# CC834/Heterogeneous-OpenCL-Image-Processing-Engine

Measured on AMD Instinct MI355X. Metric: images_per_sec, higher is better.
Workload: dtype u8

## Files before the change

heterogeneous-opencl-image-processing-engine_amd/__init__.py:

```python
from __future__ import annotations

import ctypes as C
import os
import re
import subprocess

PKG_DIR = os.path.dirname(os.path.abspath(__file__))
ROOT = os.path.dirname(PKG_DIR)
CSRC = os.path.join(PKG_DIR, "csrc")
APPS = os.path.join(PKG_DIR, "apps")
LIB_PATH = os.path.join(PKG_DIR, "libmi_blur.so")
HEADER = os.path.join(ROOT, "include", "mi_blur.h")
HIPCC = os.environ.get("HIPCC", "/opt/rocm/bin/hipcc")
os.environ.setdefault("HIP_FORCE_DEV_KERNARG", "0")
ARCH = "gfx950"

DEVICE_CPU = -1
VARIANT_AUTO, VARIANT_GENERIC, VARIANT_TILED, VARIANT_STREAM, VARIANT_DIRECT = 0, 1, 2, 3, 4
OK, ERR_INVALID, ERR_NO_DEVICE, ERR_NOMEM, ERR_STATE, ERR_UNSUPPORTED = 0, -1, -2, -3, -4, -5
UNIQUE_ID_BYTES = 128
SEP_MAX_RADIUS = 16
MEDIAN_MAX_RADIUS = 7
MORPH_MAX_RADIUS = 16
MORPH_ERODE, MORPH_DILATE, MORPH_GRADIENT = 0, 1, 2
# ... 319 lines not shown
        "mi_blur_warp_perspective_quad": (i, [C.POINTER(C.c_double), C.POINTER(C.c_double), C.POINTER(C.c_double)]),
        "mi_blur_warp_perspective_set_matrix": (i, [C.POINTER(WarpPerspective), C.POINTER(C.c_double), i]),
        "mi_blur_enqueue_warp_perspective": (i, [u8p, u8p, i, i, i, i, C.POINTER(WarpPerspective), vp]),
        "mi_blur_cpu_run_warp_perspective": (i, [u8p, u8p, i, i, i, i, C.POINTER(WarpPerspective), i]),
        "mi_blur_ctx_set_warp_perspective": (i, [vp, C.POINTER(WarpPerspective)]),
        "mi_blur_conv_preset": (i, [i, C.POINTER(Conv)]),
        "mi_blur_enqueue_conv": (i, [u8p, u8p, i, i, i, i, C.POINTER(Conv), vp]),
        "mi_blur_enqueue_conv_band": (i, [u8p, u8p, i, i, i, i, i, C.POINTER(Conv), vp]),
        "mi_blur_cpu_run_conv": (i, [u8p, u8p, i, i, i, i, C.POINTER(Conv), i]),
        "mi_blur_ctx_set_conv": (i, [vp, C.POINTER(Conv)]),
        "mi_blur_fill_synthetic": (None, [u8p, i, i, i, i, i, i]),
        "mi_blur_fnv1a64": (C.c_uint64, [u8p, C.c_size_t]),
        "mi_blur_debug_zc_trace": (i, [vp, C.POINTER(C.c_uint64), i, C.POINTER(i), C.POINTER(C.c_uint)]),
        "mi_blur_debug_xcd_times": (i, [C.POINTER(C.c_uint64), C.POINTER(C.c_uint64), i]),
        "mi_blur_debug_xcd_raw": (i, [C.POINTER(C.c_uint64), C.c_size_t, C.c_size_t]),
        "mi_blur_a1_partition": (None, [i, i, C.c_float, C.POINTER(i), C.POINTER(i)]),
        "mi_blur_shard_range": (None, [C.c_longlong, i, i, C.POINTER(C.c_longlong), C.POINTER(C.c_longlong)]),
        "mi_blur_a2_split": (None, [i, C.c_float, i, C.POINTER(A2Geometry)]),
        "mi_blur_band_of": (None, [i, i, i, i, C.POINTER(Band)]),
        "mi_blur_comm_unique_id": (i, [vp]),
        "mi_blur_comm_init_rank": (i, [C.POINTER(vp), i, i, vp]),
        "mi_blur_comm_init_all": (i, [C.POINTER(vp), i, C.POINTER(i)]),
        "mi_blur_comm_init_p2p": (i, [C.POINTER(vp), i, C.POINTER(i)]),
        "mi_blur_comm_init_pull": (i, [C.POINTER(vp), i, C.POINTER(i)]),
        "mi_blur_comm_destroy": (None, [vp]),
        "mi_blur_comm_info": (i, [vp, C.POINTER(i), C.POINTER(i), C.POINTER(i)]),
        "mi_blur_halo_exchange": (i, [vp, u8p, i, i, i, i, vp]),
        "mi_blur_peer_export": (i, [vp, vp, C.POINTER(C.c_uint64)]),
        "mi_blur_peer_open": (i, [vp, C.c_uint64, C.POINTER(vp)]),
        "mi_blur_peer_close": (i, [vp, C.c_uint64]),
# ... 471 lines not shown
```

heterogeneous-opencl-image-processing-engine_amd/csrc/blur_kernels.hip:

```cpp
#include "kernel_common.h"

#include <math.h>
#include <stdlib.h>
#include <string.h>
#include <mutex>
#include <algorithm>

namespace mi_blur {

__device__ __forceinline__ u16x2 as_pk(uint32_t x) { return __builtin_bit_cast(u16x2, x); }
__device__ __forceinline__ uint32_t as_u32(u16x2 x) { return __builtin_bit_cast(uint32_t, x); }

constexpr uint32_t EVEN_MASK = 0x00ff00ffu;
__device__ __forceinline__ uint32_t even_of(uint32_t x) { return x & EVEN_MASK; }
__device__ __forceinline__ uint32_t odd_of(uint32_t x) { return __builtin_amdgcn_perm(0u, x, 0x0c030c01u); }
__device__ __forceinline__ uint32_t mad6(uint32_t c, uint32_t t) { return as_u32(as_pk(c) * (unsigned short)6 + as_pk(t)); }

constexpr uint32_t sel_left(int C, int q)
{
    uint32_t s = 0;
    for (int j = 0; j < 4; j++) {
        int p = -4 * q + j;
        int idx = ((p % C) + C) % C;
        s |= (uint32_t)idx << (8 * j);
// ... 118 lines not shown
        h[0] = hsum_raw<C, R, 0, 0>(w); h[1] = hsum_raw<C, R, 0, 1>(w);
        h[2] = hsum_raw<C, R, 0, 2>(w); h[3] = hsum_raw<C, R, 0, 3>(w);
        h[4] = hsum_raw<C, R, 1, 0>(w); h[5] = hsum_raw<C, R, 1, 1>(w);
        h[6] = hsum_raw<C, R, 1, 2>(w); h[7] = hsum_raw<C, R, 1, 3>(w);
        return;
    }
    uint32_t Ew[8], Ow[8];
#pragma unroll
    for (int j = 0; j < 8; j++) { Ew[j] = even_of(w[j]); Ow[j] = odd_of(w[j]); }
    h[0] = hsum<C, R, 0, 0>(Ew, Ow); h[1] = hsum<C, R, 0, 1>(Ew, Ow);
    h[2] = hsum<C, R, 0, 2>(Ew, Ow); h[3] = hsum<C, R, 0, 3>(Ew, Ow);
    h[4] = hsum<C, R, 1, 0>(Ew, Ow); h[5] = hsum<C, R, 1, 1>(Ew, Ow);
    h[6] = hsum<C, R, 1, 2>(Ew, Ow); h[7] = hsum<C, R, 1, 3>(Ew, Ow);
}

struct TiledParams {
    const uint8_t *in;
    uint8_t *out;
    long long in_stride, out_stride;
    int pitch, cpr;
    int H, y0, y1;
    int ncols, nstrips;
    int TH, ntiles_y, ngroups;
    unsigned nblocks;
    int xcd;
    int debug_copy;
    unsigned long long *xcd_times;
    int tail;
};

struct __attribute__((packed, aligned(1))) Unaligned16 { u32x4 v; };
struct __attribute__((packed, aligned(1))) Unaligned8 { u32x2 v; };
struct __attribute__((packed, aligned(1))) Unaligned4 { uint32_t v; };
struct __attribute__((packed, aligned(1))) Unaligned2 { uint16_t v; };

__device__ __forceinline__ void store16_write_through(uint8_t *q, u32x4 v);
__device__ __forceinline__ void store_chunk_ragged_wt(uint8_t *q, u32x4 v, int n);
template <bool WT = false>
__device__ __forceinline__ void store_chunk_ragged(uint8_t *q, u32x4 v, int n)
{
    if constexpr (WT) { store_chunk_ragged_wt(q, v, n); return; }
    if (n >= 16) { reinterpret_cast<Unaligned16 *>(q)->v = v; return; }
    if (n & 8) { u32x2 t; t.x = v.x; t.y = v.y; reinterpret_cast<Unaligned8 *>(q)->v = t; q += 8; v.x = v.z; v.y = v.w; }
    if (n & 4) { reinterpret_cast<Unaligned4 *>(q)->v = v.x; q += 4; v.x = v.y; }
// ... 151 lines not shown
constexpr unsigned XCD_DEBUG_SLOTS = 1u << 20;
__device__ __forceinline__ void xcd_time_mark(unsigned long long *t, unsigned long long t0)
{
    if (threadIdx.x == 0 && blockIdx.x < XCD_DEBUG_SLOTS) {
        unsigned id;
        asm volatile("s_getreg_b32 %0, hwreg(HW_REG_XCC_ID)" : "=s"(id));
        t[2u * blockIdx.x] = ((unsigned long long)__builtin_amdgcn_s_memrealtime() << 4) | (id & 7u);
        t[2u * blockIdx.x + 1] = t0;
    }
}

template <int C, int R, int RPG, bool DMA, bool SHFL = false, bool RAG = false>
__global__ __launch_bounds__(256) void blur_tiled_kernel(const TiledParams p)
{
    const unsigned long long t0 = p.xcd_times ? __builtin_amdgcn_s_memrealtime() : 0ull;
    tiled_tile<C, R, RPG, DMA, SHFL, RAG>(p, xcd_map(blockIdx.x, p.nblocks, p.xcd));
    if (p.xcd_times) xcd_time_mark(p.xcd_times, t0);
}

template <int C, int R, int RPG>
__global__ __launch_bounds__(256) void blur_tiled_loop_kernel(const TiledParams p)
{
    for (unsigned L = blockIdx.x; L < p.nblocks; L += gridDim.x) {
        tiled_tile<C, R, RPG, true, false, false>(p, L);
        __syncthreads();
    }
}

template <int C, int R, int RPG, int X>
__global__ __launch_bounds__(256) void blur_tiled_x_kernel(const TiledParams p)
{
    tiled_tile<C, R, RPG, true, false, false, false, X>(p, xcd_map(blockIdx.x, p.nblocks, p.xcd));
}

struct FusedParams {
    unsigned *count;
    unsigned kcount;
    unsigned tiles_per_batch;
    int release;
    unsigned window;
    unsigned *tail_ctr;
    unsigned nstatic, ntail, nextra;
    unsigned *gate;
    unsigned gate_block, gate_seq;
};

template <int C, int R, int RPG>
__global__ __launch_bounds__(256) void blur_fused_kernel(const TiledParams p, const FusedParams f)
{
    const unsigned tpw = f.tiles_per_batch * f.window;
    const unsigned wnd = blockIdx.x / tpw, base = wnd * tpw;
    const unsigned nw = min(tpw, p.nblocks - base);
    const unsigned w = blockIdx.x - base;
    const unsigned tile = base + (nw >= 16 ? xcd_map(w, nw, p.xcd) : w);
    const unsigned b = tile / f.tiles_per_batch;
    tiled_tile<C, R, RPG, true, false, false, true>(p, tile);
    asm volatile("s_waitcnt vmcnt(0)" ::: "memory");
    __syncthreads();
    if (threadIdx.x == 0) {
        if (f.release) __hip_atomic_fetch_add(&f.count[b * f.kcount + ((w ^ (w >> 3)) & (f.kcount - 1u))], 1u, __ATOMIC_RELEASE, __HIP_MEMORY_SCOPE_AGENT);
        else __hip_atomic_fetch_add(&f.count[b * f.kcount + ((w ^ (w >> 3)) & (f.kcount - 1u))], 1u, __ATOMIC_RELAXED, __HIP_MEMORY_SCOPE_AGENT);
    }
}

template <int C, int R, int RPG, bool RAG = false>
__global__ __launch_bounds__(256) void blur_fused_tail_kernel(const TiledParams p, const FusedParams f)
{
    const unsigned long long t0 = p.xcd_times ? __builtin_amdgcn_s_memrealtime() : 0ull;
    if (f.gate && blockIdx.x == f.gate_block && threadIdx.x == 0) __hip_atomic_store(f.gate, f.gate_seq, __ATOMIC_RELAXED, __HIP_MEMORY_SCOPE_AGENT);
    unsigned tile, w;
    if (blockIdx.x >= f.nstatic) {
        __shared__ unsigned s_ticket;
        if (threadIdx.x == 0) {
            const unsigned t = __hip_atomic_fetch_add(f.tail_ctr, 1u, __ATOMIC_RELAXED, __HIP_MEMORY_SCOPE_AGENT);
            if (t == f.nextra - 1u) __hip_atomic_store(f.tail_ctr, 0u, __ATOMIC_RELAXED, __HIP_MEMORY_SCOPE_AGENT);
            s_ticket = t;
        }
        __syncthreads();
        const unsigned t = __builtin_amdgcn_readfirstlane(s_ticket);
        if (t >= f.ntail) return;
        tile = f.nstatic + t;
        w = t;
    } else {
        const unsigned tpw = f.tiles_per_batch * f.window;
// ... 380 lines not shown
    }
    wait_vmcnt<0>();
}

struct DirectParams {
    const uint8_t *in;
    uint8_t *out;
    long long in_stride, out_stride;
    long long total;
    int pitch, cpr;
    int H, y0, y1;
    int nbands;
    unsigned nblocks;
    int xcd;
    const uint8_t *top, *bottom;
};

template <int C, int R, int BH, bool PEER = false>
__global__ __launch_bounds__(256) void blur_direct_kernel(const DirectParams p)
{
    constexpr int WIN = 2 * R + 1, NR = BH + 2 * R;
    const int lane = threadIdx.x & 63, wave = threadIdx.x >> 6;
    const unsigned B = xcd_map(blockIdx.x, p.nblocks, p.xcd);
    const long long fl = (long long)(B * 4u + (unsigned)wave) * 62 - 1 + lane;
    const bool inrange = fl >= 0 && fl < p.total;
    const unsigned f = (unsigned)(fl < 0 ? 0 : (fl >= p.total ? p.total - 1 : fl));
    const unsigned col = f % (unsigned)p.cpr, t2 = f / (unsigned)p.cpr;
    const unsigned band = t2 % (unsigned)p.nbands;
    const long long img = (long long)(t2 / (unsigned)p.nbands);
    const bool compute = inrange && lane >= 1 && lane <= 62;
// ... 9 lines not shown
    if constexpr (PEER) outside = __builtin_amdgcn_ballot_w64(row0 - R < p.y0 || row0 + BH + R > p.y1) != 0ull;
    if (outside) {
#pragma unroll
        for (int j = 0; j < NR; j++) {
            const int sr = min(max(row0 - R + j, 0), p.H - 1);
            const uint8_t *rp = src + (size_t)sr * (size_t)p.pitch;
            if (sr < p.y0 && p.top) rp = p.top + (size_t)col * 16u + (size_t)sr * (size_t)p.pitch;
            if (sr >= p.y1 && p.bottom) rp = p.bottom + (size_t)col * 16u + (size_t)(sr - p.y1) * (size_t)p.pitch;
            rows[j] = *reinterpret_cast<const uint4 *>(rp);
        }
    } else {
#pragma unroll
        for (int j = 0; j < NR; j++)
            rows[j] = *reinterpret_cast<const uint4 *>(src + (size_t)min(max(row0 - R + j, 0), p.H - 1) * (size_t)p.pitch);
    }

    uint32_t hw[WIN][8];
#pragma unroll
    for (int j = 0; j < NR; j++) {
        uint32_t w[8];
        const uint4 c = rows[j];
        w[2] = c.x; w[3] = c.y; w[4] = c.z; w[5] = c.w;
        w[0] = __builtin_amdgcn_update_dpp(0u, c.z, 0x138, 0xf, 0xf, false);
        w[1] = __builtin_amdgcn_update_dpp(0u, c.w, 0x138, 0xf, 0xf, false);
        w[6] = __builtin_amdgcn_update_dpp(0u, c.x, 0x130, 0xf, 0xf, false);
        w[7] = __builtin_amdgcn_update_dpp(0u, c.y, 0x130, 0xf, 0xf, false);
        hrow_window<C, R, rowpass_default<R>>(w, any_edge, at_start, at_end, hw[j % WIN]);
        if (j >= 2 * R) {
            const int i = j - 2 * R;
            uint32_t o[4];
// ... 3 lines not shown
                    const uint32_t se = (((hw[(j + 2) % WIN][q] << 1) + hw[(j + 1) % WIN][q]) + hw[j % WIN][q]) << 4;
                    const uint32_t so = (((hw[(j + 2) % WIN][4 + q] << 1) + hw[(j + 1) % WIN][4 + q]) + hw[j % WIN][4 + q]) << 4;
                    o[q] = __builtin_amdgcn_perm(so, se, 0x07030501u);
                } else {
                    const uint32_t se = mad6(hw[(j + 3) % WIN][q], ((hw[(j + 2) % WIN][q] + hw[(j + 4) % WIN][q]) << 2) + (hw[(j + 1) % WIN][q] + hw[j % WIN][q]));
                    const uint32_t so = mad6(hw[(j + 3) % WIN][4 + q], ((hw[(j + 2) % WIN][4 + q] + hw[(j + 4) % WIN][4 + q]) << 2) + (hw[(j + 1) % WIN][4 + q] + hw[j % WIN][4 + q]));
                    o[q] = __builtin_amdgcn_perm(so, se, 0x07030501u);
                }
            }
            if (i < rows_out) {
                u32x4 v; v.x = o[0]; v.y = o[1]; v.z = o[2]; v.w = o[3];
                *reinterpret_cast<u32x4 *>(dst + (size_t)i * (size_t)p.pitch) = v;
            }
        }
    }
}

struct GenericParams {
    const uint8_t *in;
    uint8_t *out;
    long long in_stride, out_stride, total;
    int width, channels, pitch;
    int H, y0;
};

template <int R>
__global__ __launch_bounds__(256) void blur_generic_kernel(const GenericParams p)
{
    constexpr int T1[3] = {1, 2, 1};
    constexpr int T2[5] = {1, 4, 6, 4, 1};
// ... 167 lines not shown
    const long long nblocks = (long long)d.n_images * p.ntiles_y * p.nstrips;
    if (nblocks > 0x7fffffffLL) return MI_BLUR_ERR_INVALID;
    p.nblocks = (unsigned)nblocks;
    int xmap = 0;
    if (tun.xcd_remap && nblocks >= 16) {
        xmap = tun.xcd_run >= 2 ? tun.xcd_run : 1;
        if (xmap >= 2 && (long long)xmap * 8 > nblocks) xmap = 1;
    }
    p.xcd = xmap;
    p.debug_copy = tun.debug_copy;
    p.xcd_times = tun.debug_xcd_times ? debug_xcd_buffer() : nullptr;
    p.tail = pitch % 16 ? pitch % 16 : 16;
    *block_threads = (unsigned)((p.ncols * p.ngroups + 63) / 64 * 64);
    *lds_bytes = (size_t)(p.TH + 2 * R) * (p.ncols + 2) * 16;
    return rpg;
}

static int launch_tiled(const LaunchDesc &d, const Tunables &tun, bool ragged = false, const FusedDesc *fused = nullptr)
{
    if (!(fused && fused->geometry_only))
        g_last_kernel = fused ? "blur_fused_kernel" : (d.max_blocks > 0 && !ragged && d.channels <= 4 ? "blur_tiled_loop_kernel" : "blur_tiled_kernel");
    const int R = d.filter->radius;
    TiledParams p{};
    unsigned threads = 0;
    size_t lds = 0;
    const int rpg = tiled_geometry(d, tun, ragged, fused != nullptr, (fused && ragged) ? 8 : 0, p, &threads, &lds);
    if (rpg < 0) return rpg;
    const long long nblocks = p.nblocks;
    const dim3 grid((unsigned)nblocks), block(threads);
    if (fused) {
// ... 12 lines not shown
        if (fused->counters_per_batch) *fused->counters_per_batch = k;
        if (fused->tiles_per_batch) *fused->tiles_per_batch = (unsigned)tpb;
        if (fused->waves_per_block) *fused->waves_per_block = 1;
        if (fused->total_blocks) *fused->total_blocks = (unsigned)nblocks;
        const unsigned ntail = tun.fused_tail > 0 && fused->tail_ctr && nblocks >= 8192 ? (unsigned)(nblocks * tun.fused_tail / 1000) : 0u;
        if (fused->tail_tiles) *fused->tail_tiles = ntail >= 8 ? ntail : 0u;
        if (fused->geometry_only) return MI_BLUR_OK;
        p.debug_copy = 0;
        if (ntail >= 8) {
            f.tail_ctr = fused->tail_ctr; f.ntail = ntail; f.nstatic = (unsigned)nblocks - ntail;
            f.nextra = ntail + (unsigned)((long long)ntail * std::max(10, tun.fused_tail_blocks) / 100);
            g_last_kernel = "blur_fused_tail_kernel";
            const dim3 tgrid(f.nstatic + f.nextra);
            if (fused->gate && tun.fused_overlap > 0 && !ragged) {
                const long long ahead = nblocks * tun.fused_overlap / 1000;
                f.gate = fused->gate; f.gate_seq = fused->seq;
                f.gate_block = (unsigned)std::min<long long>(std::max<long long>(nblocks - ahead, 0), (long long)tgrid.x - 1);
            }
            if (p.xcd_times && tgrid.x <= 65536u) p.xcd_times += 2ull * 65536ull * (fused->seq & 15u);
            return dispatch<1, 2>(R, [&](auto Rc) { return launch_fused_r<Rc>(d, p, f, tgrid, block, lds, rpg, ragged); });
        }
        if (ragged) {
            if (!fused->tail_ctr) return MI_BLUR_ERR_UNSUPPORTED;
            f.tail_ctr = fused->tail_ctr; f.ntail = 0; f.nstatic = (unsigned)nblocks; f.nextra = 0;
            g_last_kernel = "blur_fused_tail_kernel";
        }
        return dispatch<1, 2>(R, [&](auto Rc) { return launch_fused_r<Rc>(d, p, f, grid, block, lds, rpg, ragged); });
    }
    return dispatch<1, 2>(R, [&](auto Rc) {
        return launch_tiled_r<Rc>(d, p, grid, block, lds, rpg, tun.stage_dma != 0, ragged, tun.row_shuffle != 0, tun.experiment);
    });
}

int zc_fill_batch(const LaunchDesc &d, ZcGeometry *geo, ZcBatch *b, unsigned *n_tiles)
{
    if (!geo || !b || !d.in || !d.out || d.n_images <= 0) return MI_BLUR_ERR_INVALID;
    Tunables tun = tunables();
    const bool aligned = tiled_eligible(d.in, d.out, d.width, d.channels) && !(d.in_stride % 16) && !(d.out_stride % 16);
    const long long pitch_b = (long long)d.width * d.channels;
    const bool dense = (!d.in_stride || d.in_stride == pitch_b * d.band_rows) && (!d.out_stride || d.out_stride == pitch_b * (d.y1 - d.y0));
    const bool ragged = !aligned && tun.ragged && ragged_eligible(d.width, d.channels) && dense;
    if (!aligned && !ragged) return MI_BLUR_ERR_UNSUPPORTED;
// ... 92 lines not shown
        return dispatch<1, 2>(d.filter->radius, [&](auto R) { return do_launch(blur_stream_kernel<C, R>, grid, block, lds, d, p); });
    });
}

template <int BH>
static int launch_direct_bh(const LaunchDesc &d, const Tunables &tun)
{
    g_last_kernel = "blur_direct_kernel";
    DirectParams p{};
    fill_band(p, d);
    p.cpr = p.pitch / 16; p.y1 = d.y1;
    const dim3 grid = direct_grid(p, d, BH), block(256);
    if (p.total >= 0x7fffffffLL) return MI_BLUR_ERR_INVALID;
    p.xcd = (tun.xcd_remap && p.nblocks >= 16) ? 1 : 0;
    const bool peer = d.halo_top || d.halo_bottom;
    if constexpr (BH != 8) {
        if (peer) return MI_BLUR_ERR_INVALID;
        return dispatch<1, 2>(d.filter->radius, [&](auto R) { return do_launch(blur_direct_kernel<3, R, BH>, grid, block, 0, d, p); });
    } else {
        if (peer) {
            p.top = d.halo_top; p.bottom = d.halo_bottom;
            g_last_kernel = "blur_direct_kernel (peer halo rows)";
            return dispatch<1, 2, 3, 4>(d.channels, [&](auto C) {
                return dispatch<1, 2>(d.filter->radius, [&](auto R) { return do_launch(blur_direct_kernel<C, R, 8, true>, grid, block, 0, d, p); });
            });
        }
        return dispatch<1, 2, 3, 4>(d.channels, [&](auto C) {
            return dispatch<1, 2>(d.filter->radius, [&](auto R) { return do_launch(blur_direct_kernel<C, R, 8>, grid, block, 0, d, p); });
        });
    }
// ... 80 lines not shown
```

heterogeneous-opencl-image-processing-engine_amd/csrc/blur_launch.h:

```cpp
#pragma once
#include <hip/hip_runtime.h>
#include <stdint.h>

#include "filter.h"

namespace mi_blur {

struct LaunchDesc {
    const Filter *filter;
    const uint8_t *in;
    uint8_t *out;
    int width, band_rows, channels;
    int n_images;
    int y0, y1;
    long long in_stride, out_stride;
    int concurrent;
    int max_blocks;
    int variant;
    const uint8_t *halo_top, *halo_bottom;
    hipStream_t stream;
    hipEvent_t start, stop;
};

int launch(const LaunchDesc &d);
int launch_sep(const LaunchDesc &d);
int launch_median(const LaunchDesc &d);
int launch_morph(const LaunchDesc &d);
int launch_bilateral(const LaunchDesc &d);
int launch_conv(const LaunchDesc &d);
int launch_sep_down(const LaunchDesc &d);
int launch_resize(const LaunchDesc &d);
int launch_warp(const LaunchDesc &d);
int launch_warp_persp(const LaunchDesc &d);
void set_last_kernel(const char *name);

struct Tunables;
// ... 60 lines not shown
    int stage_dma; int rpg; int xcd_remap; int debug_copy; int row_shuffle; int prefer_stream; int stream_bh; int zero_copy; int ragged;
    int fused_release;
    int experiment;
    int xcd_run;
    int zero_copy_streams;
    int zero_copy_blocks;
    int stream_updown;
    int prefer_direct;
    int direct_bh;
    int debug_xcd_times;
    int fused_window;
    int fused_tail;
    int fused_adds_per_word;
    int fused_tail_blocks;
    int fused_overlap;
    int zero_copy_server;
    int zero_copy_server_min_kb;
    int staged_server;
    int zero_copy_workers;
    int zero_copy_idle_us;
    int zero_copy_budget;
    int zero_copy_tickets;
    int resident_place_trials;
    int zero_copy_spin;
    int zero_copy_trace;
    int zero_copy_debug_base;
    int zero_copy_events;
};
enum class KnobKind { FLAG, RANGE, ONE_OF };
struct Knob { const char *key; int Tunables::*field; KnobKind kind; int lo, hi, def; const char *env; };
// ... 7 lines not shown
    {"prefer_stream", &Tunables::prefer_stream, KnobKind::FLAG, 0, 1, 0, nullptr},
    {"zero_copy", &Tunables::zero_copy, KnobKind::FLAG, 0, 1, 1, nullptr},
    {"ragged_tiled", &Tunables::ragged, KnobKind::FLAG, 0, 1, 1, nullptr},
    {"stream_band_rows", &Tunables::stream_bh, KnobKind::RANGE, 0, 4096, 0, nullptr},
    {"fused_release", &Tunables::fused_release, KnobKind::FLAG, 0, 1, 0, nullptr},
    {"experiment", &Tunables::experiment, KnobKind::FLAG, 0, 1, 0, nullptr},
    {"stream_updown", &Tunables::stream_updown, KnobKind::FLAG, 0, 1, 1, nullptr},
    {"zero_copy_streams", &Tunables::zero_copy_streams, KnobKind::RANGE, 1, 8, 4, nullptr},
    {"zero_copy_blocks", &Tunables::zero_copy_blocks, KnobKind::RANGE, 0, 1 << 20, 24, nullptr},
    {"prefer_direct", &Tunables::prefer_direct, KnobKind::RANGE, 0, 2, 1, "MI_BLUR_DIRECT"},
    {"direct_bh", &Tunables::direct_bh, KnobKind::ONE_OF, knob_bits(4, 8, 12, 16), 0, 8, nullptr},
    {"fused_adds_per_word", &Tunables::fused_adds_per_word, KnobKind::RANGE, 4, 4096, 32, nullptr},
    {"fused_tail_blocks", &Tunables::fused_tail_blocks, KnobKind::RANGE, 10, 800, 25, nullptr},
    {"fused_tail", &Tunables::fused_tail, KnobKind::RANGE, 0, 500, 30, "MI_BLUR_FUSED_TAIL"},
    {"fused_overlap", &Tunables::fused_overlap, KnobKind::RANGE, 0, 500, 30, "MI_BLUR_FUSED_OVERLAP"},
    {"fused_window", &Tunables::fused_window, KnobKind::RANGE, 1, 4096, 8, nullptr},
    {"debug_xcd_times", &Tunables::debug_xcd_times, KnobKind::FLAG, 0, 1, 0, nullptr},
    {"zero_copy_events", &Tunables::zero_copy_events, KnobKind::FLAG, 0, 1, 1, nullptr},
    {"zero_copy_server", &Tunables::zero_copy_server, KnobKind::FLAG, 0, 1, 1, nullptr},
    {"staged_server", &Tunables::staged_server, KnobKind::FLAG, 0, 1, 1, "MI_BLUR_STAGED_SERVER"},
    {"zero_copy_server_min_kb", &Tunables::zero_copy_server_min_kb, KnobKind::RANGE, 0, 1 << 20, 1280, nullptr},
    {"zero_copy_trace", &Tunables::zero_copy_trace, KnobKind::FLAG, 0, 1, 0, nullptr},
    {"zero_copy_tickets", &Tunables::zero_copy_tickets, KnobKind::FLAG, 0, 1, 1, nullptr},
    {"zero_copy_spin", &Tunables::zero_copy_spin, KnobKind::FLAG, 0, 1, 0, nullptr},
    {"zero_copy_debug_base", &Tunables::zero_copy_debug_base, KnobKind::RANGE, 0, 1 << 20, 0, nullptr},
    {"resident_place_trials", &Tunables::resident_place_trials, KnobKind::RANGE, 0, 8, 4, "MI_BLUR_PLACE_TRIALS"},
    {"zero_copy_workers", &Tunables::zero_copy_workers, KnobKind::RANGE, 1, 2048, 48, nullptr},
    {"zero_copy_idle_us", &Tunables::zero_copy_idle_us, KnobKind::RANGE, 10, 100000, 300, nullptr},
    {"zero_copy_budget", &Tunables::zero_copy_budget, KnobKind::RANGE, 1, 1 << 20, 256, nullptr},
    {"xcd_run", &Tunables::xcd_run, KnobKind::RANGE, 0, 1 << 20, 0, nullptr},
// ... 19 lines not shown
```

heterogeneous-opencl-image-processing-engine_amd/csrc/mi_blur_api.cpp:

```cpp
#include "api_internal.h"
#include "blur_launch.h"
#include "cpu_device.h"

#include <sched.h>
#include <time.h>

#include <algorithm>
#include <chrono>
#include <climits>
#include <cmath>
#include <cstdio>
#include <cstdlib>
#include <cstring>
#include <mutex>
#include <new>
#include <deque>
#include <functional>
#include <condition_variable>
#include <thread>
#include <vector>

using namespace mi_blur;

__attribute__((constructor)) static void mi_blur_runtime_defaults() { setenv("HIP_FORCE_DEV_KERNARG", "0", 0); }
// ... 571 lines not shown
    }
    void wait(CpuJob *j)
    {
        std::unique_lock<std::mutex> lk(m);
        cv_done.wait(lk, [&] { return j->done; });
    }
    ~CpuWorker()
    {
        { std::lock_guard<std::mutex> lk(m); stop = true; }
        cv_work.notify_all();
        if (th.joinable()) th.join();
    }
};

}

struct mi_blur_ctx {
    int device = 0, W = 0, H = 0, C = 0, max_batch = 0, n_threads = 0;
    Filter filter{};
    size_t image_bytes = 0;
    std::vector<Slot> slots;
    int next_slot = 0;
    mi_blur_timing tm{};
    uint8_t *pool_in = nullptr, *pool_out = nullptr;
    int pool_images = 0;
    long long cursor = 0;
    int rr = 0;
    std::vector<TimedLaunch> ev_pool;
    size_t ev_used = 0;
    uint64_t timed_launches = 0, timed_bytes_alg = 0;
// ... 2 lines not shown
    bool zc_ref_valid = false;
    double zc_covered_ms = 0.0;
    unsigned *fused_count = nullptr, *fused_host = nullptr;
    int fused_cap = 0, fused_batches = 0;
    unsigned fused_tpb = 0, fused_wpb = 0, fused_blocks = 0;
    unsigned fused_k = 8;
    int fused_n = 0, fused_batch = 0;
    unsigned fused_passes = 0;
    hipStream_t fused_poll = nullptr;
    unsigned long long *fused_word = nullptr, *fused_word_dev = nullptr;
    unsigned fused_watch_seq = 0;
    bool fused_watched = false;
    bool fused_watch_busy = false;
    hipStream_t fused_second = nullptr;
    hipEvent_t fused_ev = nullptr;
    unsigned fused_seq = 0;
    bool fused_gated = false;
    bool fused_on_second = false;
    bool fused_second_busy = false;
    ZcServer *zc = nullptr;
    std::vector<float> place_ms;
    int place_kept = 0;
    std::vector<CpuJob *> cpu_jobs;
    CpuWorker *cpu_worker = nullptr;
    bool submitted = false;
    bool is_cpu() const { return device == MI_BLUR_DEVICE_CPU; }
};

static bool is_pinned(const void *p)
{
    hipPointerAttribute_t a;
    if (hipPointerGetAttributes(&a, p) != hipSuccess) { (void)hipGetLastError(); return false; }
    return a.type == hipMemoryTypeHost;
}
// ... 275 lines not shown
    if (c->is_cpu()) {
        for (CpuJob *j : c->cpu_jobs) {
            c->cpu_worker->wait(j);
            c->tm.kernel_ms += j->ms;
            delete j;
        }
        c->cpu_jobs.clear();
    } else {
        HIP_TRY(hipSetDevice(c->device));
        for (auto &s : c->slots) {
            int rc = finish_slot(c, s);
            if (rc) return rc;
        }
        for (auto &s : c->slots) HIP_TRY(hipStreamSynchronize(s.stream));
        if (c->fused_second) HIP_TRY(hipStreamSynchronize(c->fused_second));
        c->fused_second_busy = false; c->fused_gated = false;
        c->fused_watch_busy = false;
        harvest_resident(c);
        c->zc_ref_valid = false;
    }
    if (timing) *timing = c->tm;
    return MI_BLUR_OK;
}

extern "C" int mi_blur_get_timing(mi_blur_ctx *c, mi_blur_timing *timing)
{
    if (!c || !timing) return MI_BLUR_ERR_INVALID;
    *timing = c->tm;
    return MI_BLUR_OK;
}

// ... 27 lines not shown
            if (getenv("MI_BLUR_DEBUG_SERVER"))
                fprintf(stderr, "[mi_blur] destroy: server state head %u launched %u servers_done %u tail %u; stream query %d\n", z.head, z.launched,
                        z.ctl ? z.ctl->servers_done : 0u, z.ctl ? z.ctl->tail : 0u, z.stream ? (int)hipStreamQuery(z.stream) : -1);
            if (z.stream) { (void)hipStreamSynchronize(z.stream); (void)hipStreamDestroy(z.stream); }
            if (getenv("MI_BLUR_DEBUG_SERVER")) fprintf(stderr, "[mi_blur] destroy: servers gone\n");
            if (z.dev) (void)hipFree(z.dev);
            if (z.trace) (void)hipFree(z.trace);
            if (z.ctl) (void)hipHostFree(z.ctl);
            delete c->zc;
            c->zc = nullptr;
        }
        for (auto &s : c->slots) free_slot(s);
        for (auto &t : c->ev_pool) { (void)hipEventDestroy(t.s); (void)hipEventDestroy(t.e); }
        if (c->zc_ref) (void)hipEventDestroy(c->zc_ref);
        if (c->fused_count) (void)hipFree(c->fused_count);
        if (c->fused_host) (void)hipHostFree(c->fused_host);
        if (c->fused_poll) { (void)hipStreamSynchronize(c->fused_poll); (void)hipStreamDestroy(c->fused_poll); }
        if (c->fused_word) (void)hipHostFree(c->fused_word);
        if (c->fused_second) (void)hipStreamDestroy(c->fused_second);
        if (c->fused_ev) (void)hipEventDestroy(c->fused_ev);
        if (c->pool_in) (void)hipFree(c->pool_in);
        if (c->pool_out) (void)hipFree(c->pool_out);
        (void)hipGetLastError();
    }
    delete c;
}

static int zc_server_submit(mi_blur_ctx *c, Slot &s, const LaunchDesc &d, const Tunables &tun)
{
    if (c->filter.kind != FilterKind::BOX) return MI_BLUR_ERR_UNSUPPORTED;
// ... 530 lines not shown
    return MI_BLUR_OK;
}

extern "C" void *mi_blur_resident_in(mi_blur_ctx *c) { return c ? c->pool_in : nullptr; }
extern "C" void *mi_blur_resident_out(mi_blur_ctx *c) { return c ? c->pool_out : nullptr; }

static int fused_join(mi_blur_ctx *c)
{
    if (!c->fused_second_busy) return MI_BLUR_OK;
    HIP_TRY(hipEventRecord(c->fused_ev, c->fused_second));
    for (auto &s : c->slots) HIP_TRY(hipStreamWaitEvent(s.stream, c->fused_ev, 0));
    c->fused_second_busy = false;
    return MI_BLUR_OK;
}

extern "C" int mi_blur_resident_run(mi_blur_ctx *c, int n_images, int batch, int timed_every)
{
    if (!c || n_images < 0 || batch <= 0) return MI_BLUR_ERR_INVALID;
    if (c->filter.kind != FilterKind::BOX) return MI_BLUR_ERR_UNSUPPORTED;
    if (c->is_cpu() || !c->pool_in) return MI_BLUR_ERR_STATE;
    if (batch > c->pool_images) return MI_BLUR_ERR_INVALID;
    HIP_TRY(hipSetDevice(c->device));
    { int rc = fused_join(c); if (rc) return rc; }
    int launch_idx = 0;
    for (int done = 0; done < n_images; done += batch, launch_idx++) {
        const int b = std::min(batch, n_images - done);
        const bool timed = timed_every > 0 && launch_idx % timed_every == 0;
        if (c->cursor + b > c->pool_images) c->cursor = 0;
        Slot &s = c->slots[c->rr];
        c->rr = (c->rr + 1) % (int)c->slots.size();
        LaunchDesc d = ctx_launch(c, c->pool_in + (size_t)c->cursor * c->image_bytes, c->pool_out + (size_t)c->cursor * c->image_bytes,
                                  c->H, b, 0, c->H);
        d.stream = s.stream;
        d.concurrent = (int)c->slots.size();
        if (timed) {
            if (c->ev_used == c->ev_pool.size()) {
                TimedLaunch t{};
                HIP_TRY(hipEventCreate(&t.s));
                HIP_TRY(hipEventCreate(&t.e));
                c->ev_pool.push_back(t);
            }
            d.start = c->ev_pool[c->ev_used].s; d.stop = c->ev_pool[c->ev_used].e;
            c->ev_used++;
        }
        int rc = launch(d);
        if (rc) return rc;
        c->cursor += b;
        c->tm.launches += 1;
        if (timed) { c->timed_launches += 1; c->timed_bytes_alg += 2ull * c->image_bytes * (uint64_t)b; }
    }
    c->tm.images += (uint64_t)n_images;
    c->tm.bytes_alg += 2ull * c->image_bytes * (uint64_t)n_images;
    return MI_BLUR_OK;
}

static size_t fused_words(int cap) { return 8 * (size_t)cap + 16384; }
constexpr size_t FUSED_TAIL_BANK = 32, FUSED_GATE_WORD = 64, FUSED_EXTRA_WORDS = 96;

extern "C" int mi_blur_resident_run_fused(mi_blur_ctx *c, int n_images, int batch, int timed)
{
    if (!c || n_images <= 0 || batch <= 0) return MI_BLUR_ERR_INVALID;
    if (c->filter.kind != FilterKind::BOX) return MI_BLUR_ERR_UNSUPPORTED;
    if (c->is_cpu() || !c->pool_in) return MI_BLUR_ERR_STATE;
    if (n_images > c->pool_images) return MI_BLUR_ERR_INVALID;
    HIP_TRY(hipSetDevice(c->device));
    const int nb = (n_images + batch - 1) / batch;
    if (nb > c->fused_cap) {
        for (auto &s : c->slots) HIP_TRY(hipStreamSynchronize(s.stream));
        if (c->fused_second) HIP_TRY(hipStreamSynchronize(c->fused_second));
        c->fused_second_busy = false; c->fused_gated = false;
        if (c->fused_count) { (void)hipFree(c->fused_count); c->fused_count = nullptr; }
        if (c->fused_host) { (void)hipHostFree(c->fused_host); c->fused_host = nullptr; }
        c->fused_cap = 0;
        const int cap = std::max(nb, c->pool_images);
        HIP_TRY(hipMalloc((void **)&c->fused_count, sizeof(unsigned) * (fused_words(cap) + FUSED_EXTRA_WORDS)));
        HIP_TRY(hipMemset(c->fused_count + fused_words(cap), 0, sizeof(unsigned) * FUSED_EXTRA_WORDS));
        HIP_TRY(hipMemcpy(c->fused_count + fused_words(cap) + FUSED_GATE_WORD, &c->fused_seq, sizeof(unsigned), hipMemcpyHostToDevice));
        HIP_TRY(hipDeviceSynchronize());
        HIP_TRY(hipHostMalloc((void **)&c->fused_host, sizeof(unsigned) * fused_words(cap), hipHostMallocDefault));
        c->fused_cap = cap;
        c->fused_passes = 0;
    }
    if (!c->fused_poll) {
        HIP_TRY(hipStreamCreateWithFlags(&c->fused_poll, hipStreamNonBlocking));
        HIP_TRY(hipMemcpyAsync(c->fused_host, c->fused_count, sizeof(unsigned) * fused_words(c->fused_cap), hipMemcpyDeviceToHost, c->fused_poll));
        HIP_TRY(hipStreamSynchronize(c->fused_poll));
    }
    if (c->cursor + n_images > c->pool_images) c->cursor = 0;
    Slot &s = c->slots[0];
    LaunchDesc d = ctx_launch(c, c->pool_in + (size_t)c->cursor * c->image_bytes, c->pool_out + (size_t)c->cursor * c->image_bytes,
                              c->H, n_images, 0, c->H);
    d.variant = MI_BLUR_VARIANT_TILED; d.stream = s.stream;
    const Tunables tun = tunables();
    unsigned tpb = 0, wpb = 0, blocks = 0, kcnt = 8, ntail = 0;
    unsigned *const extra = c->fused_count + fused_words(c->fused_cap);
    const unsigned seq = c->fused_seq + 1u;
    FusedDesc f{c->fused_count, batch, &tpb, &wpb, &blocks, &tun, true, extra + (tun.fused_overlap > 0 ? (seq & 1u) * FUSED_TAIL_BANK : 0), (long long)fused_words(c->fused_cap), &kcnt,
                &ntail, nullptr, seq};
    int rc = launch_fused(d, f);
    if (rc) return rc;
    const bool same = n_images == c->fused_n && batch == c->fused_batch && tpb == c->fused_tpb && wpb == c->fused_wpb && kcnt == c->fused_k &&
                      blocks == c->fused_blocks && c->fused_passes > 0 && c->fused_passes < (1u << 20);
    const bool raises = tun.fused_overlap > 0 && ntail > 0 && !(timed & 2) && tiled_eligible(d.in, d.out, c->W, c->C);
    const bool overlap = raises && same && c->fused_gated;
    if (overlap) {
        d.stream = c->fused_on_second ? s.stream : c->fused_second;
        rc = launch_fused_gate(extra + FUSED_GATE_WORD, c->fused_seq, d.stream);
        if (rc) return rc;
    } else {
        rc = fused_join(c);
        if (rc) return rc;
    }
    if (raises) f.gate = extra + FUSED_GATE_WORD;
    if (same) {
        c->fused_passes += 1;
    } else {
        if (c->fused_watch_busy) { HIP_TRY(hipStreamSynchronize(c->fused_second)); c->fused_watch_busy = false; }
        HIP_TRY(hipMemsetAsync(c->fused_count, 0, sizeof(unsigned) * (size_t)kcnt * (size_t)nb, s.stream));
        c->fused_n = n_images; c->fused_batch = batch; c->fused_passes = 1;
        c->fused_tpb = tpb; c->fused_wpb = wpb; c->fused_blocks = blocks; c->fused_k = kcnt;
    }
    c->fused_batches = nb;
    c->fused_watched = false;
    if (timed & 2) {
        if (c->fused_passes == 1) HIP_TRY(hipStreamSynchronize(s.stream));
        if (!c->fused_word) {
            HIP_TRY(hipHostMalloc((void **)&c->fused_word, sizeof(unsigned long long), hipHostMallocDefault));
            *c->fused_word = 0;
            HIP_TRY(hipHostGetDevicePointer((void **)&c->fused_word_dev, c->fused_word, 0));
        }
    }
    if (timed & 1) {
        if (c->ev_used == c->ev_pool.size()) {
            TimedLaunch t{};
            HIP_TRY(hipEventCreate(&t.s));
            HIP_TRY(hipEventCreate(&t.e));
            c->ev_pool.push_back(t);
        }
        d.start = c->ev_pool[c->ev_used].s; d.stop = c->ev_pool[c->ev_used].e;
        c->ev_used++;
    }
    f.geometry_only = false;
    rc = launch_fused(d, f);
    if (rc) { c->fused_passes = 0; c->fused_batches = 0; c->fused_gated = false; return rc; }
    c->fused_seq = seq;
    c->fused_gated = raises;
    c->fused_on_second = d.stream == c->fused_second;
    if (c->fused_on_second) c->fused_second_busy = true;
    c->cursor += n_images;
    c->tm.launches += 1;
    c->tm.images += (uint64_t)n_images;
    c->tm.bytes_alg += 2ull * c->image_bytes * (uint64_t)n_images;
    if (timed & 1) { c->timed_launches += 1; c->timed_bytes_alg += 2ull * c->image_bytes * (uint64_t)n_images; }
    if (timed & 2) {
        c->fused_watch_seq += 1;
        rc = launch_fused_watch(c->fused_count, (unsigned)nb, tpb, blocks, wpb * c->fused_passes, c->fused_word_dev, c->fused_watch_seq, c->fused_second, c->fused_k);
        if (rc) return rc;
        c->fused_watched = true;
        c->fused_watch_busy = true;
        c->fused_second_busy = true;
    }
    return MI_BLUR_OK;
}
// ... 215 lines not shown
```

include/mi_blur.h:

```cpp
#ifndef MI_BLUR_H
#define MI_BLUR_H

#include <stddef.h>
#include <stdint.h>

#ifdef __cplusplus
extern "C" {
#endif

#define MI_BLUR_VERSION 1
#define MI_BLUR_DEVICE_CPU (-1)

typedef enum mi_blur_status {
    MI_BLUR_OK = 0,
    MI_BLUR_ERR_INVALID = -1,
    MI_BLUR_ERR_NO_DEVICE = -2,
    MI_BLUR_ERR_NOMEM = -3,
    MI_BLUR_ERR_STATE = -4,
    MI_BLUR_ERR_UNSUPPORTED = -5,
    MI_BLUR_ERR_HIP_BASE = -1000,
    MI_BLUR_ERR_RCCL_BASE = -2000
} mi_blur_status;

typedef enum mi_blur_variant {
// ... 228 lines not shown
} mi_blur_conv_preset_id;
int mi_blur_conv_preset(int preset, mi_blur_conv *k);

int mi_blur_enqueue_conv(const uint8_t *d_in, uint8_t *d_out, int width, int height, int channels, int n_images,
                         const mi_blur_conv *k, void *stream);
int mi_blur_enqueue_conv_band(const uint8_t *d_in, uint8_t *d_out, int width, int band_rows, int channels,
                              int out_row_begin, int out_row_end, const mi_blur_conv *k, void *stream);
int mi_blur_cpu_run_conv(const uint8_t *in, uint8_t *out, int width, int height, int channels, int n_images,
                         const mi_blur_conv *k, int n_threads);
int mi_blur_ctx_set_conv(mi_blur_ctx *ctx, const mi_blur_conv *k);

int mi_blur_debug_xcd_times(uint64_t end_ticks[8], uint64_t begin_ticks[8], int rearm);

int mi_blur_debug_xcd_raw(uint64_t *out, size_t first_slot, size_t n_slots);

int mi_blur_debug_zc_trace(mi_blur_ctx *ctx, uint64_t *out, int max_batches, int *n_workers, unsigned *batches_published);

void mi_blur_fill_synthetic(uint8_t *host, int width, int height, int channels,
                            int first_index, int n_images, int n_threads);
uint64_t mi_blur_fnv1a64(const uint8_t *host, size_t n);

void mi_blur_a1_partition(int mode, int batch_count, float gpu_ratio, int *n_cpu, int *n_gpu);
void mi_blur_shard_range(long long n_units, int g, int G, long long *begin, long long *end);

typedef struct mi_blur_a2_geometry {
    int split_row;
    int cpu_input_rows, cpu_output_rows;
    int gpu_input_rows, gpu_output_rows;
} mi_blur_a2_geometry;
void mi_blur_a2_split(int height, float gpu_ratio, int halo, mi_blur_a2_geometry *g);
// ... 38 lines not shown
```

Measured before the change: 15.35 million.

## Extend gated cross-pass overlap to plain tiled and direct blur passes

Generalizes the fused-path gate mechanism into a shared PassGate that plain tiled and direct blur kernels raise from a block near the end of their grid. When one batch covers all images, the next resident pass launches on an alternate stream behind a gate wait instead of joining, so consecutive passes overlap their tails and heads. The gate word moves to its own allocation and the sequence and stream state is unified across fused and plain passes. This adds dual-stream ordering complexity and relies on pass-to-pass independence of the buffers.

```diff
diff --git a/heterogeneous-opencl-image-processing-engine_amd/__init__.py b/heterogeneous-opencl-image-processing-engine_amd/__init__.py
--- a/heterogeneous-opencl-image-processing-engine_amd/__init__.py
+++ b/heterogeneous-opencl-image-processing-engine_amd/__init__.py
@@ -357,6 +357,7 @@
         "mi_blur_debug_zc_trace": (i, [vp, C.POINTER(C.c_uint64), i, C.POINTER(i), C.POINTER(C.c_uint)]),
         "mi_blur_debug_xcd_times": (i, [C.POINTER(C.c_uint64), C.POINTER(C.c_uint64), i]),
         "mi_blur_debug_xcd_raw": (i, [C.POINTER(C.c_uint64), C.c_size_t, C.c_size_t]),
+        "mi_blur_debug_pass_state": (i, [vp, C.POINTER(C.c_uint), C.POINTER(i), C.POINTER(i)]),
         "mi_blur_a1_partition": (None, [i, i, C.c_float, C.POINTER(i), C.POINTER(i)]),
         "mi_blur_shard_range": (None, [C.c_longlong, i, i, C.POINTER(C.c_longlong), C.POINTER(C.c_longlong)]),
         "mi_blur_a2_split": (None, [i, C.c_float, i, C.POINTER(A2Geometry)]),
diff --git a/heterogeneous-opencl-image-processing-engine_amd/csrc/blur_kernels.hip b/heterogeneous-opencl-image-processing-engine_amd/csrc/blur_kernels.hip
--- a/heterogeneous-opencl-image-processing-engine_amd/csrc/blur_kernels.hip
+++ b/heterogeneous-opencl-image-processing-engine_amd/csrc/blur_kernels.hip
@@ -156,6 +156,15 @@
     h[6] = hsum<C, R, 1, 2>(Ew, Ow); h[7] = hsum<C, R, 1, 3>(Ew, Ow);
 }
 
+struct PassGate { unsigned *word; unsigned block, seq; };
+__device__ __forceinline__ void pass_gate_raise(const PassGate &g)
+{
+    if (__builtin_expect(blockIdx.x == g.block, 0)) {
+        asm volatile("" ::: "memory");
+        if (g.word && threadIdx.x == 0) __hip_atomic_store(g.word, g.seq, __ATOMIC_RELAXED, __HIP_MEMORY_SCOPE_AGENT);
+    }
+}
+
 struct TiledParams {
     const uint8_t *in;
     uint8_t *out;
@@ -167,9 +176,13 @@
     unsigned nblocks;
     int xcd;
     int debug_copy;
+    unsigned gate_block;
     unsigned long long *xcd_times;
     int tail;
+    unsigned gate_seq;
+    unsigned *gate_word;
 };
+static_assert(sizeof(TiledParams) + 14 <= 128, "blockDim.x must stay within the first two 64-byte lines of the kernel arguments");
 
 struct __attribute__((packed, aligned(1))) Unaligned16 { u32x4 v; };
 struct __attribute__((packed, aligned(1))) Unaligned8 { u32x2 v; };
@@ -351,6 +364,7 @@
 __global__ __launch_bounds__(256) void blur_tiled_kernel(const TiledParams p)
 {
     const unsigned long long t0 = p.xcd_times ? __builtin_amdgcn_s_memrealtime() : 0ull;
+    if constexpr (!RAG) pass_gate_raise(PassGate{p.gate_word, p.gate_block, p.gate_seq});
     tiled_tile<C, R, RPG, DMA, SHFL, RAG>(p, xcd_map(blockIdx.x, p.nblocks, p.xcd));
     if (p.xcd_times) xcd_time_mark(p.xcd_times, t0);
 }
@@ -378,8 +392,7 @@
     unsigned window;
     unsigned *tail_ctr;
     unsigned nstatic, ntail, nextra;
-    unsigned *gate;
-    unsigned gate_block, gate_seq;
+    PassGate gate;
 };
 
 template <int C, int R, int RPG>
@@ -404,7 +417,7 @@
 __global__ __launch_bounds__(256) void blur_fused_tail_kernel(const TiledParams p, const FusedParams f)
 {
     const unsigned long long t0 = p.xcd_times ? __builtin_amdgcn_s_memrealtime() : 0ull;
-    if (f.gate && blockIdx.x == f.gate_block && threadIdx.x == 0) __hip_atomic_store(f.gate, f.gate_seq, __ATOMIC_RELAXED, __HIP_MEMORY_SCOPE_AGENT);
+    pass_gate_raise(f.gate);
     unsigned tile, w;
     if (blockIdx.x >= f.nstatic) {
         __shared__ unsigned s_ticket;
@@ -815,6 +828,8 @@
     unsigned nblocks;
     int xcd;
     const uint8_t *top, *bottom;
+    unsigned long long *xcd_times;
+    PassGate gate;
 };
 
 template <int C, int R, int BH, bool PEER = false>
@@ -854,6 +869,8 @@
         for (int j = 0; j < NR; j++)
             rows[j] = *reinterpret_cast<const uint4 *>(src + (size_t)min(max(row0 - R + j, 0), p.H - 1) * (size_t)p.pitch);
     }
+    const unsigned long long t0 = p.xcd_times ? __builtin_amdgcn_s_memrealtime() : 0ull;
+    if constexpr (!PEER) pass_gate_raise(p.gate);
 
     uint32_t hw[WIN][8];
 #pragma unroll
@@ -887,6 +904,7 @@
             }
         }
     }
+    if (p.xcd_times) xcd_time_mark(p.xcd_times, t0);
 }
 
 struct GenericParams {
@@ -1084,6 +1102,19 @@
     *block_threads = (unsigned)((p.ncols * p.ngroups + 63) / 64 * 64);
     *lds_bytes = (size_t)(p.TH + 2 * R) * (p.ncols + 2) * 16;
     return rpg;
+}
+
+constexpr int PLAIN_OVERLAP_TILED = 10, PLAIN_OVERLAP_DIRECT = 90;
+static void plain_gate(const LaunchDesc &d, const Tunables &tun, int kernel_default, unsigned nblocks, PassGate &g, unsigned long long *&stamps)
+{
+    if (!d.gate) return;
+    if (stamps && nblocks <= 65536u) stamps += 2ull * 65536ull * (d.pass_seq & 15u);
+    const int v = tun.plain_overlap < 0 ? kernel_default : tun.plain_overlap;
+    const bool dense = (!d.in_stride || d.in_stride == dense_in(d)) && (!d.out_stride || d.out_stride == dense_out(d));
+    if (v <= 0 || !dense || d.max_blocks > 0 || d.halo_top || d.halo_bottom || (long long)nblocks < tun.plain_overlap_min_blocks) return;
+    const long long ahead = (long long)nblocks * v / 1000;
+    g = PassGate{d.gate, (unsigned)std::min<long long>(std::max<long long>((long long)nblocks - ahead, 0), (long long)nblocks - 1), d.pass_seq};
+    if (d.gated) *d.gated = true;
 }
 
 static int launch_tiled(const LaunchDesc &d, const Tunables &tun, bool ragged = false, const FusedDesc *fused = nullptr)
@@ -1126,8 +1157,7 @@
             const dim3 tgrid(f.nstatic + f.nextra);
             if (fused->gate && tun.fused_overlap > 0 && !ragged) {
                 const long long ahead = nblocks * tun.fused_overlap / 1000;
-                f.gate = fused->gate; f.gate_seq = fused->seq;
-                f.gate_block = (unsigned)std::min<long long>(std::max<long long>(nblocks - ahead, 0), (long long)tgrid.x - 1);
+                f.gate = PassGate{fused->gate, (unsigned)std::min<long long>(std::max<long long>(nblocks - ahead, 0), (long long)tgrid.x - 1), fused->seq};
             }
             if (p.xcd_times && tgrid.x <= 65536u) p.xcd_times += 2ull * 65536ull * (fused->seq & 15u);
             return dispatch<1, 2>(R, [&](auto Rc) { return launch_fused_r<Rc>(d, p, f, tgrid, block, lds, rpg, ragged); });
@@ -1138,6 +1168,11 @@
             g_last_kernel = "blur_fused_tail_kernel";
         }
         return dispatch<1, 2>(R, [&](auto Rc) { return launch_fused_r<Rc>(d, p, f, grid, block, lds, rpg, ragged); });
+    }
+    if (!ragged && !tun.experiment) {
+        PassGate g{};
+        plain_gate(d, tun, PLAIN_OVERLAP_TILED, p.nblocks, g, p.xcd_times);
+        p.gate_word = g.word; p.gate_block = g.block; p.gate_seq = g.seq;
     }
     return dispatch<1, 2>(R, [&](auto Rc) {
         return launch_tiled_r<Rc>(d, p, grid, block, lds, rpg, tun.stage_dma != 0, ragged, tun.row_shuffle != 0, tun.experiment);
@@ -1260,6 +1295,8 @@
     if (p.total >= 0x7fffffffLL) return MI_BLUR_ERR_INVALID;
     p.xcd = (tun.xcd_remap && p.nblocks >= 16) ? 1 : 0;
     const bool peer = d.halo_top || d.halo_bottom;
+    p.xcd_times = tun.debug_xcd_times ? debug_xcd_buffer() : nullptr;
+    if (!peer) plain_gate(d, tun, PLAIN_OVERLAP_DIRECT, p.nblocks, p.gate, p.xcd_times);
     if constexpr (BH != 8) {
         if (peer) return MI_BLUR_ERR_INVALID;
         return dispatch<1, 2>(d.filter->radius, [&](auto R) { return do_launch(blur_direct_kernel<3, R, BH>, grid, block, 0, d, p); });
diff --git a/heterogeneous-opencl-image-processing-engine_amd/csrc/blur_launch.h b/heterogeneous-opencl-image-processing-engine_amd/csrc/blur_launch.h
--- a/heterogeneous-opencl-image-processing-engine_amd/csrc/blur_launch.h
+++ b/heterogeneous-opencl-image-processing-engine_amd/csrc/blur_launch.h
@@ -20,6 +20,9 @@
     const uint8_t *halo_top, *halo_bottom;
     hipStream_t stream;
     hipEvent_t start, stop;
+    unsigned *gate;
+    unsigned pass_seq;
+    bool *gated;
 };
 
 int launch(const LaunchDesc &d);
@@ -110,6 +113,8 @@
     int fused_adds_per_word;
     int fused_tail_blocks;
     int fused_overlap;
+    int plain_overlap;
+    int plain_overlap_min_blocks;
     int zero_copy_server;
     int zero_copy_server_min_kb;
     int staged_server;
@@ -147,6 +152,8 @@
     {"fused_tail_blocks", &Tunables::fused_tail_blocks, KnobKind::RANGE, 10, 800, 25, nullptr},
     {"fused_tail", &Tunables::fused_tail, KnobKind::RANGE, 0, 500, 30, "MI_BLUR_FUSED_TAIL"},
     {"fused_overlap", &Tunables::fused_overlap, KnobKind::RANGE, 0, 500, 30, "MI_BLUR_FUSED_OVERLAP"},
+    {"plain_overlap", &Tunables::plain_overlap, KnobKind::RANGE, -1, 500, -1, "MI_BLUR_PLAIN_OVERLAP"},
+    {"plain_overlap_min_blocks", &Tunables::plain_overlap_min_blocks, KnobKind::RANGE, 1, 1 << 30, 8192, nullptr},
     {"fused_window", &Tunables::fused_window, KnobKind::RANGE, 1, 4096, 8, nullptr},
     {"debug_xcd_times", &Tunables::debug_xcd_times, KnobKind::FLAG, 0, 1, 0, nullptr},
     {"zero_copy_events", &Tunables::zero_copy_events, KnobKind::FLAG, 0, 1, 1, nullptr},
diff --git a/heterogeneous-opencl-image-processing-engine_amd/csrc/mi_blur_api.cpp b/heterogeneous-opencl-image-processing-engine_amd/csrc/mi_blur_api.cpp
--- a/heterogeneous-opencl-image-processing-engine_amd/csrc/mi_blur_api.cpp
+++ b/heterogeneous-opencl-image-processing-engine_amd/csrc/mi_blur_api.cpp
@@ -609,6 +609,8 @@
 };
 
 }
+
+enum { PASS_NONE = 0, PASS_FUSED = 1, PASS_PLAIN = 2 };
 
 struct mi_blur_ctx {
     int device = 0, W = 0, H = 0, C = 0, max_batch = 0, n_threads = 0;
@@ -641,10 +643,15 @@
     bool fused_watch_busy = false;
     hipStream_t fused_second = nullptr;
     hipEvent_t fused_ev = nullptr;
-    unsigned fused_seq = 0;
-    bool fused_gated = false;
-    bool fused_on_second = false;
+    unsigned *pass_gate = nullptr;
+    unsigned pass_seq = 0;
+    int pass_kind = PASS_NONE;
+    bool pass_gated = false;
+    bool pass_on_second = false;
     bool fused_second_busy = false;
+    int plain_n = 0;
+    const char *plain_kernel = nullptr;
+    Tunables plain_tun{};
     ZcServer *zc = nullptr;
     std::vector<float> place_ms;
     int place_kept = 0;
@@ -950,7 +957,7 @@
         }
         for (auto &s : c->slots) HIP_TRY(hipStreamSynchronize(s.stream));
         if (c->fused_second) HIP_TRY(hipStreamSynchronize(c->fused_second));
-        c->fused_second_busy = false; c->fused_gated = false;
+        c->fused_second_busy = false; c->pass_gated = false;
         c->fused_watch_busy = false;
         harvest_resident(c);
         c->zc_ref_valid = false;
@@ -1008,6 +1015,7 @@
         for (auto &t : c->ev_pool) { (void)hipEventDestroy(t.s); (void)hipEventDestroy(t.e); }
         if (c->zc_ref) (void)hipEventDestroy(c->zc_ref);
         if (c->fused_count) (void)hipFree(c->fused_count);
+        if (c->pass_gate) (void)hipFree(c->pass_gate);
         if (c->fused_host) (void)hipHostFree(c->fused_host);
         if (c->fused_poll) { (void)hipStreamSynchronize(c->fused_poll); (void)hipStreamDestroy(c->fused_poll); }
         if (c->fused_word) (void)hipHostFree(c->fused_word);
@@ -1568,6 +1576,42 @@
     return MI_BLUR_OK;
 }
 
+static int pass_gate_word(mi_blur_ctx *c)
+{
+    if (c->pass_gate) return MI_BLUR_OK;
+    HIP_TRY(hipMalloc((void **)&c->pass_gate, 128));
+    HIP_TRY(hipMemset(c->pass_gate, 0, 128));
+    HIP_TRY(hipMemcpy(c->pass_gate, &c->pass_seq, sizeof(unsigned), hipMemcpyHostToDevice));
+    HIP_TRY(hipDeviceSynchronize());
+    return MI_BLUR_OK;
+}
+
+static int pass_begin(mi_blur_ctx *c, bool overlap, hipStream_t *stream)
+{
+    if (overlap && c->pass_gated && c->pass_gate) {
+        *stream = c->pass_on_second ? c->slots[0].stream : c->fused_second;
+        return launch_fused_gate(c->pass_gate, c->pass_seq, *stream);
+    }
+    *stream = c->slots[0].stream;
+    return fused_join(c);
+}
+
+static void pass_issued(mi_blur_ctx *c, int kind, unsigned seq, bool raises, hipStream_t stream)
+{
+    c->pass_kind = kind; c->pass_seq = seq; c->pass_gated = raises;
+    c->pass_on_second = stream == c->fused_second;
+    if (c->pass_on_second) c->fused_second_busy = true;
+}
+
+extern "C" int mi_blur_debug_pass_state(mi_blur_ctx *c, unsigned *pass_number, int *on_second_stream, int *raises_gate)
+{
+    if (!c) return MI_BLUR_ERR_INVALID;
+    if (pass_number) *pass_number = c->pass_seq;
+    if (on_second_stream) *on_second_stream = c->pass_on_second ? 1 : 0;
+    if (raises_gate) *raises_gate = c->pass_gated ? 1 : 0;
+    return MI_BLUR_OK;
+}
+
 extern "C" int mi_blur_resident_run(mi_blur_ctx *c, int n_images, int batch, int timed_every)
 {
     if (!c || n_images < 0 || batch <= 0) return MI_BLUR_ERR_INVALID;
@@ -1575,7 +1619,21 @@
     if (c->is_cpu() || !c->pool_in) return MI_BLUR_ERR_STATE;
     if (batch > c->pool_images) return MI_BLUR_ERR_INVALID;
     HIP_TRY(hipSetDevice(c->device));
-    { int rc = fused_join(c); if (rc) return rc; }
+    const Tunables tun = tunables();
+    const bool whole = n_images > 0 && batch >= n_images && c->slots.size() == 1 && tun.plain_overlap != 0;
+    hipStream_t pass_stream = nullptr;
+    bool gated = false, like = false;
+    if (whole) {
+        int rc = pass_gate_word(c);
+        if (rc) return rc;
+        like = c->pass_kind == PASS_PLAIN && c->plain_n == n_images && !memcmp(&c->plain_tun, &tun, sizeof tun);
+        rc = pass_begin(c, like, &pass_stream);
+        if (rc) return rc;
+    } else {
+        int rc = fused_join(c);
+        if (rc) return rc;
+        c->pass_gated = false; c->pass_kind = PASS_NONE;
+    }
     int launch_idx = 0;
     for (int done = 0; done < n_images; done += batch, launch_idx++) {
         const int b = std::min(batch, n_images - done);
@@ -1586,6 +1644,7 @@
         LaunchDesc d = ctx_launch(c, c->pool_in + (size_t)c->cursor * c->image_bytes, c->pool_out + (size_t)c->cursor * c->image_bytes,
                                   c->H, b, 0, c->H);
         d.stream = s.stream;
+        if (whole) { d.stream = pass_stream; d.gate = c->pass_gate; d.pass_seq = c->pass_seq + 1u; d.gated = &gated; }
         d.concurrent = (int)c->slots.size();
         if (timed) {
             if (c->ev_used == c->ev_pool.size()) {
@@ -1598,7 +1657,12 @@
             c->ev_used++;
         }
         int rc = launch(d);
-        if (rc) return rc;
+        if (rc) { c->pass_gated = false; return rc; }
+        if (whole) {
+            const char *kernel = last_kernel();
+            pass_issued(c, PASS_PLAIN, d.pass_seq, gated && (!like || kernel == c->plain_kernel), d.stream);
+            c->plain_n = n_images; c->plain_kernel = kernel; c->plain_tun = tun;
+        }
         c->cursor += b;
         c->tm.launches += 1;
         if (timed) { c->timed_launches += 1; c->timed_bytes_alg += 2ull * c->image_bytes * (uint64_t)b; }
@@ -1609,7 +1673,7 @@
 }
 
 static size_t fused_words(int cap) { return 8 * (size_t)cap + 16384; }
-constexpr size_t FUSED_TAIL_BANK = 32, FUSED_GATE_WORD = 64, FUSED_EXTRA_WORDS = 96;
+constexpr size_t FUSED_TAIL_BANK = 32, FUSED_EXTRA_WORDS = 64;
 
 extern "C" int mi_blur_resident_run_fused(mi_blur_ctx *c, int n_images, int batch, int timed)
 {
@@ -1622,14 +1686,13 @@
     if (nb > c->fused_cap) {
         for (auto &s : c->slots) HIP_TRY(hipStreamSynchronize(s.stream));
         if (c->fused_second) HIP_TRY(hipStreamSynchronize(c->fused_second));
-        c->fused_second_busy = false; c->fused_gated = false;
+        c->fused_second_busy = false; c->pass_gated = false;
         if (c->fused_count) { (void)hipFree(c->fused_count); c->fused_count = nullptr; }
         if (c->fused_host) { (void)hipHostFree(c->fused_host); c->fused_host = nullptr; }
         c->fused_cap = 0;
         const int cap = std::max(nb, c->pool_images);
         HIP_TRY(hipMalloc((void **)&c->fused_count, sizeof(unsigned) * (fused_words(cap) + FUSED_EXTRA_WORDS)));
         HIP_TRY(hipMemset(c->fused_count + fused_words(cap), 0, sizeof(unsigned) * FUSED_EXTRA_WORDS));
-        HIP_TRY(hipMemcpy(c->fused_count + fused_words(cap) + FUSED_GATE_WORD, &c->fused_seq, sizeof(unsigned), hipMemcpyHostToDevice));
         HIP_TRY(hipDeviceSynchronize());
         HIP_TRY(hipHostMalloc((void **)&c->fused_host, sizeof(unsigned) * fused_words(cap), hipHostMallocDefault));
         c->fused_cap = cap;
@@ -1648,7 +1711,7 @@
     const Tunables tun = tunables();
     unsigned tpb = 0, wpb = 0, blocks = 0, kcnt = 8, ntail = 0;
     unsigned *const extra = c->fused_count + fused_words(c->fused_cap);
-    const unsigned seq = c->fused_seq + 1u;
+    const unsigned seq = c->pass_seq + 1u;
     FusedDesc f{c->fused_count, batch, &tpb, &wpb, &blocks, &tun, true, extra + (tun.fused_overlap > 0 ? (seq & 1u) * FUSED_TAIL_BANK : 0), (long long)fused_words(c->fused_cap), &kcnt,
                 &ntail, nullptr, seq};
     int rc = launch_fused(d, f);
@@ -1656,16 +1719,10 @@
     const bool same = n_images == c->fused_n && batch == c->fused_batch && tpb == c->fused_tpb && wpb == c->fused_wpb && kcnt == c->fused_k &&
                       blocks == c->fused_blocks && c->fused_passes > 0 && c->fused_passes < (1u << 20);
     const bool raises = tun.fused_overlap > 0 && ntail > 0 && !(timed & 2) && tiled_eligible(d.in, d.out, c->W, c->C);
-    const bool overlap = raises && same && c->fused_gated;
-    if (overlap) {
-        d.stream = c->fused_on_second ? s.stream : c->fused_second;
-        rc = launch_fused_gate(extra + FUSED_GATE_WORD, c->fused_seq, d.stream);
-        if (rc) return rc;
-    } else {
-        rc = fused_join(c);
-        if (rc) return rc;
-    }
-    if (raises) f.gate = extra + FUSED_GATE_WORD;
+    if (raises) { rc = pass_gate_word(c); if (rc) return rc; }
+    rc = pass_begin(c, raises && same && c->pass_kind == PASS_FUSED, &d.stream);
+    if (rc) return rc;
+    if (raises) f.gate = c->pass_gate;
     if (same) {
         c->fused_passes += 1;
     } else {
@@ -1696,11 +1753,8 @@
     }
     f.geometry_only = false;
     rc = launch_fused(d, f);
-    if (rc) { c->fused_passes = 0; c->fused_batches = 0; c->fused_gated = false; return rc; }
-    c->fused_seq = seq;
-    c->fused_gated = raises;
-    c->fused_on_second = d.stream == c->fused_second;
-    if (c->fused_on_second) c->fused_second_busy = true;
+    if (rc) { c->fused_passes = 0; c->fused_batches = 0; c->pass_gated = false; return rc; }
+    pass_issued(c, PASS_FUSED, seq, raises, d.stream);
     c->cursor += n_images;
     c->tm.launches += 1;
     c->tm.images += (uint64_t)n_images;
diff --git a/include/mi_blur.h b/include/mi_blur.h
--- a/include/mi_blur.h
+++ b/include/mi_blur.h
@@ -266,6 +266,8 @@
 
 int mi_blur_debug_xcd_raw(uint64_t *out, size_t first_slot, size_t n_slots);
 
+int mi_blur_debug_pass_state(mi_blur_ctx *ctx, unsigned *pass_number, int *on_second_stream, int *raises_gate);
+
 int mi_blur_debug_zc_trace(mi_blur_ctx *ctx, uint64_t *out, int max_batches, int *n_workers, unsigned *batches_published);
 
 void mi_blur_fill_synthetic(uint8_t *host, int width, int height, int channels,
```

Measured after the change: 15.01 million. 2.2% lower.
